# robingg1/PoseTraj

Measured on AMD Instinct MI355X. Metric: denoised frames/sec, higher is better.
Workload: dtype f16; 1 GPU; SVD-img2vid U-Net + controlnet_sdv, 14x576x1024, 25 Euler steps, CFG, 1 clip per GPU (BASELINE configs[2]); weights=random-init at full SVD dimensions (1524.6 M + 682.0 M params), output_finite=True, hipgraph=True, two_streams=True, rccl_world_size=1, weight_broadcast_collectives=0

## Files before the change

posetraj_amd/csrc/norm.hip:

```cpp
#include "pt_common.h"

namespace {

constexpr int GN_TX = 32, GN_TY = 8, GN_SLOTS = 36;

__global__ __launch_bounds__(256) void gn_partial_kernel(const f16* __restrict__ x0, const f16* __restrict__ x1,
                                                         int C0, int C1, int groups, int64_t rows_per_sample,
                                                         int rows_per_slab, float* __restrict__ part) {
    __shared__ float red[GN_TY][GN_TX * 8 * 2];
    __shared__ float chan[256 * 2];
    const int tx = threadIdx.x & 31, ty = threadIdx.x >> 5;
    const int slab = blockIdx.x, strip = blockIdx.y, sample = blockIdx.z;
    const int Ctot = C0 + C1, cg = Ctot / groups;
    const int c = strip * 256 + tx * 8;
    float s[8], q[8];
#pragma unroll
    for (int j = 0; j < 8; ++j) { s[j] = 0.f; q[j] = 0.f; }
    if (c < Ctot) {
        float pv[8];
#pragma unroll
        for (int j = 0; j < 8; ++j) pv[j] = pt_gn_pivot(x0, x1, C0, C1, rows_per_sample, sample, (c + j) / cg * cg);
        const f16* src; int ld, co;
        if (c < C0) { src = x0; ld = C0; co = c; } else { src = x1; ld = C1; co = c - C0; }
        const int64_t r0 = (int64_t)slab * rows_per_slab;
        int64_t r1 = r0 + rows_per_slab; if (r1 > rows_per_sample) r1 = rows_per_sample;
        const f16* base = src + ((int64_t)sample * rows_per_sample) * ld + co;
        int64_t r = r0 + ty;
        for (; r + 3 * GN_TY < r1; r += 4 * GN_TY) {
            f16x8 v[4];
#pragma unroll
            for (int u = 0; u < 4; ++u) v[u] = *(const f16x8*)(base + (r + u * GN_TY) * ld);
#pragma unroll
            for (int u = 0; u < 4; ++u)
#pragma unroll
                for (int j = 0; j < 8; ++j) { const float f = (float)v[u][j] - pv[j]; s[j] += f; q[j] += f * f; }
        }
        for (; r < r1; r += GN_TY) {
            const f16x8 v = *(const f16x8*)(base + r * ld);
#pragma unroll
            for (int j = 0; j < 8; ++j) { const float f = (float)v[j] - pv[j]; s[j] += f; q[j] += f * f; }
        }
    }
#pragma unroll
    for (int j = 0; j < 8; ++j) { red[ty][(tx * 8 + j) * 2] = s[j]; red[ty][(tx * 8 + j) * 2 + 1] = q[j]; }
    __syncthreads();
    for (int i = threadIdx.x; i < 256 * 2; i += 256) {
        float a = 0.f;
#pragma unroll
        for (int y = 0; y < GN_TY; ++y) a += red[y][i];
        chan[i] = a;
    }
    __syncthreads();
    const int c_lo = strip * 256, c_hi = (c_lo + 256 < Ctot) ? c_lo + 256 : Ctot;
    const int g_lo = c_lo / cg, g_hi = (c_hi - 1) / cg;
    const int ng = g_hi - g_lo + 1;
    if ((int)threadIdx.x < 2 * ng) {
        const int g = g_lo + (threadIdx.x >> 1), which = threadIdx.x & 1;
        int a0 = g * cg, a1 = a0 + cg;
        if (a0 < c_lo) a0 = c_lo;
        if (a1 > c_hi) a1 = c_hi;
        float acc = 0.f;
        for (int ch = a0; ch < a1; ++ch) acc += chan[(ch - c_lo) * 2 + which];
        part[((((int64_t)sample * gridDim.x + slab) * gridDim.y + strip) * GN_SLOTS + (g - g_lo)) * 2 + which] = acc;
    }
}

__device__ __forceinline__ void gn_fold_sample(const float* __restrict__ part, const f16* __restrict__ x0, const f16* __restrict__ x1,
                                               int C0, int C1, int sample, int nslabs, int nstrips, int groups,
                                               int64_t rows_per_sample, float eps, float* grp) {
    const int Ctot = C0 + C1, cg = Ctot / groups;
    const int sub = threadIdx.x & 7;
    for (int g = threadIdx.x >> 3; g < groups; g += blockDim.x >> 3) {
        float s = 0.f, q = 0.f;
        const int ch0 = g * cg, ch1 = ch0 + cg - 1;
        const float pg = pt_gn_pivot(x0, x1, C0, C1, rows_per_sample, sample, ch0);
        for (int strip = ch0 / 256; strip <= ch1 / 256; ++strip) {
            const int g_lo = (strip * 256) / cg;
            const float* base = part + ((int64_t)sample * nslabs * nstrips + strip) * GN_SLOTS * 2 + (g - g_lo) * 2;
            const int64_t step = (int64_t)nstrips * GN_SLOTS * 2;
            int sl = sub;
            for (; sl + 24 < nslabs; sl += 32) {
                const f32x2 e0 = *(const f32x2*)(base + sl * step), e1 = *(const f32x2*)(base + (sl + 8) * step);
                const f32x2 e2 = *(const f32x2*)(base + (sl + 16) * step), e3 = *(const f32x2*)(base + (sl + 24) * step);
                s += e0[0]; q += e0[1]; s += e1[0]; q += e1[1]; s += e2[0]; q += e2[1]; s += e3[0]; q += e3[1];
            }
            for (; sl < nslabs; sl += 8) {
                const float* e = base + sl * step;
                s += e[0]; q += e[1];
            }
        }
#pragma unroll
        for (int o = 1; o < 8; o <<= 1) { s += __shfl_xor(s, o); q += __shfl_xor(q, o); }
        if (sub == 0) {
            const double cnt = (double)rows_per_sample * cg;
            const double d = (double)s / cnt;
            double var = (double)q / cnt - d * d;
            if (var < 0.0) var = 0.0;
            grp[4 * g] = pg;
            grp[4 * g + 1] = (float)d;
            grp[4 * g + 2] = (float)(1.0 / sqrt(var + (double)eps));
        }
    }
}

__global__ __launch_bounds__(256) void gn_apply_kernel(const f16* __restrict__ x0, const f16* __restrict__ x1, int C0,
                                                       int C1, int rows_per_sample, int rows_per_block,
                                                       const float* __restrict__ part, int nslabs, int nstrips, int groups,
                                                       float eps, const f16* __restrict__ gamma, const f16* __restrict__ beta,
                                                       int silu, f16* __restrict__ y) {
    extern __shared__ __attribute__((aligned(16))) float s_ab[];
    __shared__ float grp[4 * 32];
    const int Ctot = C0 + C1, CH = Ctot >> 3;
    f16* const s_pv = (f16*)(s_ab + 2 * Ctot);
    const int sample = blockIdx.y;
    const int r0 = blockIdx.x * rows_per_block;
    const int r1 = min(r0 + rows_per_block, rows_per_sample);
    gn_fold_sample(part, x0, x1, C0, C1, sample, nslabs, nstrips, groups, rows_per_sample, eps, grp);
    __syncthreads();
    {
        const int cg = Ctot / groups;
        for (int c = threadIdx.x; c < Ctot; c += 256) {
            const int g = c / cg;
            const float a = grp[4 * g + 2] * (float)gamma[c];
            s_ab[2 * c] = a;
            s_ab[2 * c + 1] = (float)beta[c] - grp[4 * g + 1] * a;
            s_pv[c] = (f16)grp[4 * g];
        }
    }
    __syncthreads();
    const int64_t base_row = (int64_t)sample * rows_per_sample;
    const int dr = 256 / CH, dc = 256 - dr * CH;
    int row = r0 + (int)threadIdx.x / CH, c = (int)threadIdx.x % CH;
    auto advance = [&](int& rw, int& cc) {
        rw += dr; cc += dc;
        if (cc >= CH) { cc -= CH; ++rw; }
    };
    auto load = [&](int rw, int cc) -> f16x8 {
        const int ch = cc * 8;
        const int64_t grow = base_row + rw;
        return ch < C0 ? *(const f16x8*)(x0 + grow * C0 + ch) : *(const f16x8*)(x1 + grow * C1 + (ch - C0));
    };
    auto finish = [&](int rw, int cc, const f16x8& v) {
        const int ch = cc * 8;
        const f32x4* abp = (const f32x4*)(s_ab + ch * 2);
        const f16x8 pv = *(const f16x8*)(s_pv + ch);
        f16x8 o;
#pragma unroll
        for (int h = 0; h < 4; ++h) {
            const f32x4 k = abp[h];
            float u0 = ((float)v[2 * h] - (float)pv[2 * h]) * k[0] + k[1], u1 = ((float)v[2 * h + 1] - (float)pv[2 * h + 1]) * k[2] + k[3];
            if (silu) { u0 = pt_silu(u0); u1 = pt_silu(u1); }
            o[2 * h] = (f16)u0; o[2 * h + 1] = (f16)u1;
        }
        *(f16x8*)(y + (base_row + rw) * Ctot + ch) = o;
    };
    for (;;) {
        int rw[4], cc[4];
        rw[0] = row; cc[0] = c;
#pragma unroll
        for (int u = 1; u < 4; ++u) { rw[u] = rw[u - 1]; cc[u] = cc[u - 1]; advance(rw[u], cc[u]); }
        if (rw[3] >= r1) break;
        f16x8 v[4];
#pragma unroll
        for (int u = 0; u < 4; ++u) v[u] = load(rw[u], cc[u]);
#pragma unroll
        for (int u = 0; u < 4; ++u) finish(rw[u], cc[u], v[u]);
        row = rw[3]; c = cc[3];
        advance(row, c);
    }
    for (; row < r1; advance(row, c)) finish(row, c, load(row, c));
}

template <int NCH>
__global__ __launch_bounds__(256) void layernorm_kernel(const f16* __restrict__ x, int64_t M, int C,
                                                        const f16* __restrict__ vec, int ldv, int vec_mode, int vG,
                                                        const f16* __restrict__ gamma, const f16* __restrict__ beta,
                                                        float eps, f16* __restrict__ y) {
    const int lane = threadIdx.x & 63;
    const int64_t row = (int64_t)blockIdx.x * 4 + (threadIdx.x >> 6);
    if (row >= M) return;
    const int CH = C >> 3;
    float v[NCH][8];
    float sum = 0.f;
    const f16* vrow = vec_mode ? vec + (int64_t)(row / vG) * ldv : nullptr;
#pragma unroll
// ... 80 lines not shown
    if (!ok) return;
#pragma unroll
    for (int k = 0; k < CPL; ++k) {
        const int ch = l + LPR * k;
        const f16x8 g = *(const f16x8*)(gamma + ch * 8), b = *(const f16x8*)(beta + ch * 8);
        f16x8 o;
#pragma unroll
        for (int j = 0; j < 8; ++j) o[j] = (f16)((v[k][j] - mean) * rstd * (float)g[j] + (float)b[j]);
        *(f16x8*)(y + row * C + ch * 8) = o;
    }
}

int slab_rows(int64_t rows_per_sample, int nstrips, int n_samples) {
    int64_t target_slabs = 2048 / ((int64_t)nstrips * n_samples);
    if (target_slabs < 1) target_slabs = 1;
    if (target_slabs > 1024) target_slabs = 1024;
    int64_t rows = (rows_per_sample + target_slabs - 1) / target_slabs;
    if (rows < 64) rows = 64;
    rows = (rows + 7) / 8 * 8;
    return (int)rows;
}

}

extern "C" int64_t pt_groupnorm_scratch_floats(int64_t rows_total, int32_t C, int32_t n_samples) {
    const int64_t rps = rows_total / (n_samples > 0 ? n_samples : 1);
    const int nstrips = (C + 255) / 256;
    const int rows = slab_rows(rps, nstrips, n_samples);
    const int64_t nslabs = (rps + rows - 1) / rows;
    return (int64_t)n_samples * nslabs * nstrips * GN_SLOTS * 2;
}

extern "C" int pt_groupnorm_stats(const void* x0, const void* x1, int32_t C0, int32_t C1, int32_t groups,
                                  int64_t rows_per_sample, int32_t n_samples, float* partials, void* stream) {
    const int Ctot = C0 + C1;
    PT_CHECK(x0 && partials, "pt_groupnorm_stats: null pointer");
    PT_CHECK(C0 % 8 == 0 && C1 % 8 == 0 && groups > 0 && groups <= 32 && Ctot % groups == 0 && Ctot / groups >= 2,
             "pt_groupnorm_stats: C0=%d C1=%d groups=%d", C0, C1, groups);
    PT_CHECK((C1 == 0) == (x1 == nullptr), "pt_groupnorm_stats: x1/C1 mismatch");
    PT_CHECK(rows_per_sample > 0 && n_samples > 0, "pt_groupnorm_stats: empty input");
    const int nstrips = (Ctot + 255) / 256;
    const int rows = slab_rows(rows_per_sample, nstrips, n_samples);
    const int nslabs = (int)((rows_per_sample + rows - 1) / rows);
    PT_CHECK(n_samples <= 65535 && nstrips <= 65535, "pt_groupnorm_stats: grid too large");
    hipLaunchKernelGGL(gn_partial_kernel, dim3(nslabs, nstrips, n_samples), dim3(256), 0, (hipStream_t)stream, (const f16*)x0,
                       (const f16*)x1, C0, C1, groups, rows_per_sample, rows, partials);
    PT_LAUNCH_CHECK("pt_groupnorm_stats");
    return 0;
}

extern "C" int pt_groupnorm_apply(const void* x0, const void* x1, int32_t C0, int32_t C1, int32_t groups,
                                  int64_t rows_per_sample, int32_t n_samples, float eps, const void* gamma,
                                  const void* beta, const float* partials, int32_t silu, void* y, void* stream) {
    PT_CHECK(x0 && gamma && beta && partials && y, "pt_groupnorm_apply: null pointer");
    PT_CHECK(C0 % 8 == 0 && C1 % 8 == 0, "pt_groupnorm_apply: channels must be multiples of 8");
    const int Ctot = C0 + C1;
    PT_CHECK(Ctot >= 8 && Ctot <= 4096, "pt_groupnorm_apply: %d channels unsupported (8 .. 4096)", Ctot);
    PT_CHECK(groups > 0 && groups <= 32 && Ctot % groups == 0 && Ctot / groups >= 2, "pt_groupnorm_apply: C=%d groups=%d", Ctot, groups);
    PT_CHECK(rows_per_sample > 0 && rows_per_sample < (1ll << 31) && n_samples > 0 && n_samples <= 65535, "pt_groupnorm_apply: bad sizes");
    const int nstrips = (Ctot + 255) / 256;
    const int srows = slab_rows(rows_per_sample, nstrips, n_samples);
    const int nslabs = (int)((rows_per_sample + srows - 1) / srows);
    int64_t per_sample = 4096 / n_samples;
    if (per_sample < 1) per_sample = 1;
    int64_t rows_per_block = (rows_per_sample + per_sample - 1) / per_sample;
    const int64_t total_chunks = rows_per_sample * n_samples * (Ctot >> 3);
    const int min_chunks = total_chunks < (int64_t)256 * 32 * 1024 ? 8 : 32;
    const int64_t min_rows = (256 * min_chunks + (Ctot >> 3) - 1) / (Ctot >> 3);
    if (rows_per_block < min_rows) rows_per_block = min_rows;
    const unsigned bx = (unsigned)((rows_per_sample + rows_per_block - 1) / rows_per_block);
    hipLaunchKernelGGL(gn_apply_kernel, dim3(bx, (unsigned)n_samples), dim3(256), (size_t)Ctot * 10, (hipStream_t)stream,
                       (const f16*)x0, (const f16*)x1, C0, C1, (int)rows_per_sample, (int)rows_per_block, partials, nslabs,
                       nstrips, groups, eps, (const f16*)gamma, (const f16*)beta, silu, (f16*)y);
    PT_LAUNCH_CHECK("pt_groupnorm_apply");
    return 0;
}

extern "C" int pt_layernorm_f16(const void* x, int64_t M, int32_t C, const void* vec, int32_t ldv, int32_t vec_mode,
                                int32_t vG, const void* gamma, const void* beta, float eps, void* y, void* stream) {
    PT_CHECK(x && gamma && beta && y, "pt_layernorm_f16: null pointer");
    PT_CHECK(C % 8 == 0 && C <= 2048, "pt_layernorm_f16: C=%d must be a multiple of 8 and <= 2048", C);
    PT_CHECK(vec_mode == 0 || (vec_mode == 1 && vec && vG > 0 && ldv % 8 == 0), "pt_layernorm_f16: bad vec arguments");
    hipStream_t s = (hipStream_t)stream;
#define LN_NARROW(LPR, CPL)                                                                                            \
    do {                                                                                                               \
        const int64_t rpb = 4 * (64 / LPR);                                                                            \
        hipLaunchKernelGGL((layernorm_narrow_kernel<LPR, CPL>), dim3((unsigned)((M + rpb - 1) / rpb)), dim3(256), 0, s, \
                           (const f16*)x, M, C, (const f16*)vec, ldv, vec_mode, vG, (const f16*)gamma, (const f16*)beta, \
// ... 3 lines not shown
    } while (0)
    if (C == 320) LN_NARROW(8, 5);
    if (C == 640) LN_NARROW(16, 5);
    if (C == 1280) LN_NARROW(32, 5);
#undef LN_NARROW
    const unsigned blocks = (unsigned)((M + 3) / 4);
    const int nch = ((C >> 3) + 63) / 64;
#define LN_LAUNCH(NCH)                                                                                              \
    hipLaunchKernelGGL(layernorm_kernel<NCH>, dim3(blocks), dim3(256), 0, s, (const f16*)x, M, C, (const f16*)vec, \
                       ldv, vec_mode, vG, (const f16*)gamma, (const f16*)beta, eps, (f16*)y)
    if (nch == 1) LN_LAUNCH(1); else if (nch == 2) LN_LAUNCH(2); else if (nch == 3) LN_LAUNCH(3); else LN_LAUNCH(4);
#undef LN_LAUNCH
    PT_LAUNCH_CHECK("pt_layernorm_f16");
    return 0;
}
```

posetraj_amd/hip.py:

```python
from __future__ import annotations

import ctypes as C
import os
import re
import subprocess

HERE = os.path.dirname(os.path.abspath(__file__))
CSRC = os.path.join(HERE, "csrc")
LIB_PATH = os.path.abspath(os.environ["PT_LIB"]) if os.environ.get("PT_LIB") else os.path.join(HERE, "libposetraj_hip.so")
SOURCES = ["api.hip", "igemm.hip", "ffn.hip", "lnlin.hip", "norm.hip", "attn.hip", "attn_general.hip", "elementwise.hip", "vae.hip", "vae_f32.hip", "clip.hip", "raster.hip", "train.hip", "gemm.hip", "backward.hip", "attn_bwd.hip", "batch.hip", "control.hip", "sampler.hip"]
HEADERS = ["pt_common.h", "igemm_tail.h", "pt_fold.h"]
HEADER = os.path.join(HERE, "..", "include", "posetraj_hip.h")
STRUCT_CLASSES = {"pt_igemm_params": "IgemmParams", "pt_ffn_params": "FfnParams", "pt_lnlin_params": "LnLinParams",
                  "pt_conv_f32_params": "ConvF32Params", "pt_gemm_params": "GemmParams"}
OPTIM_HEADER = os.path.join(HERE, "..", "include", "posetraj_optim.h")
OPTIM_STRUCT_CLASSES = {"pt_adam8_segment": "Adam8Segment"}
DET_HEADER = os.path.join(HERE, "..", "include", "posetraj_det.h")
TEMPORAL_HEADER = os.path.join(HERE, "..", "include", "posetraj_temporal.h")
BATCH_HEADER = os.path.join(HERE, "..", "include", "posetraj_batch.h")
CONTROL_HEADER = os.path.join(HERE, "..", "include", "posetraj_control.h")
SAMPLER_HEADER = os.path.join(HERE, "..", "include", "posetraj_sampler.h")

_lib = _checked = None

_SCALARS = {"int": C.c_int, "int32_t": C.c_int32, "int64_t": C.c_int64, "float": C.c_float, "double": C.c_double}
_TYPE = r"(?:const\s+)?\w+\s*\*?"
_DECL = re.compile(r"""\s*(?: typedef\s+struct\s+(?P<tag>\w+)\s*\{(?P<body>[^{}]*)\}\s*(?P=tag)\s*;
                            | (?P<ret>%s)\s*\b(?P<fn>pt[odtbcs]?_[a-z0-9_]+)\s*\((?P<params>[^()]*)\)\s*;
                            | extern\s+"C"\s*\{ | \} )""" % _TYPE, re.X)
_FIELD = re.compile(r"(%s)\s*\b(\w+(?:\s*,\s*\w+)*)" % _TYPE)


def _ctype(spelling: str, structs: dict, returned: bool = False):
    m = re.fullmatch(r"(const\s+)?(\w+)\s*(\*)?", spelling)
    const, base, ptr = m.groups() if m else (None, None, None)
    if not ptr and not const and base in _SCALARS:
        return _SCALARS[base]
    if ptr and const and base in structs:
        return C.POINTER(structs[base])
    if ptr and const and base == "char" and returned:
        return C.c_char_p
    if ptr and (base == "void" or base in _SCALARS):
        return C.c_void_p
# ... 19 lines not shown
    structs, protos, pos = dict(known_structs or {}), {}, 0
    while text[pos:].strip():
        m = _DECL.match(text, pos)
        if not m:
            raise ValueError(f"posetraj_hip.h: cannot read the declaration {text[pos:].strip().split(';')[0][:200]!r}")
        if m.group("tag"):
            tag = m.group("tag")
            if tag not in struct_classes:
                raise ValueError(f"posetraj_hip.h: struct {tag!r} has no class name in posetraj_amd.hip.STRUCT_CLASSES")
            fields = [(n, _ctype(t, structs)) for t, n in _declarators(m.group("body"), ";")]
            structs[tag] = type(struct_classes[tag], (C.Structure,), {"_fields_": fields, "__doc__": f"``{tag}`` of include/posetraj_hip.h."})
        elif m.group("fn"):
            params = m.group("params").strip()
            protos[m.group("fn")] = (" ".join(m.group("ret").split()), [] if params == "void" else [t for t, _ in _declarators(params, ",")])
        pos = m.end()
    named = re.findall(r"pt[odtbcs]?_[a-z0-9_]+\s*\(", text)
    if len(named) != len(protos):
        raise ValueError(f"posetraj_hip.h: {len(named)} names are followed by '(' but {len(protos)} prototypes were read")
    return int(version.group(1)), {k: v for k, v in structs.items() if k not in (known_structs or {})}, protos


with open(HEADER) as _f:
    ABI_VERSION, _STRUCTS, PROTOTYPES = _parse_header(_f.read())
IgemmParams, FfnParams, LnLinParams, ConvF32Params, GemmParams = (_STRUCTS[tag] for tag in STRUCT_CLASSES)
SIGNATURES = {name: (_ctype(ret, _STRUCTS, returned=True), [_ctype(t, _STRUCTS) for t in params]) for name, (ret, params) in PROTOTYPES.items()}
with open(OPTIM_HEADER) as _f:
    OPTIM_ABI_VERSION, _OPTIM_STRUCTS, OPTIM_PROTOTYPES = _parse_header(_f.read(), OPTIM_STRUCT_CLASSES, "PT_OPTIM_ABI_VERSION")
Adam8Segment = _OPTIM_STRUCTS["pt_adam8_segment"]
OPTIM_SIGNATURES = {name: (_ctype(ret, _OPTIM_STRUCTS, returned=True), [_ctype(t, _OPTIM_STRUCTS) for t in params])
                    for name, (ret, params) in OPTIM_PROTOTYPES.items()}
with open(DET_HEADER) as _f:
    DET_ABI_VERSION, _, DET_PROTOTYPES = _parse_header(_f.read(), {}, "PT_DET_ABI_VERSION", _STRUCTS)
DET_SIGNATURES = {name: (_ctype(ret, _STRUCTS, returned=True), [_ctype(t, _STRUCTS) for t in params]) for name, (ret, params) in DET_PROTOTYPES.items()}
with open(TEMPORAL_HEADER) as _f:
    TEMPORAL_ABI_VERSION, _, TEMPORAL_PROTOTYPES = _parse_header(_f.read(), {}, "PT_TEMPORAL_ABI_VERSION", _STRUCTS)
TEMPORAL_SIGNATURES = {name: (_ctype(ret, _STRUCTS, returned=True), [_ctype(t, _STRUCTS) for t in params]) for name, (ret, params) in TEMPORAL_PROTOTYPES.items()}
with open(BATCH_HEADER) as _f:
    BATCH_ABI_VERSION, _, BATCH_PROTOTYPES = _parse_header(_f.read(), {}, "PT_BATCH_ABI_VERSION", _STRUCTS)
BATCH_SIGNATURES = {name: (_ctype(ret, _STRUCTS, returned=True), [_ctype(t, _STRUCTS) for t in params]) for name, (ret, params) in BATCH_PROTOTYPES.items()}
with open(CONTROL_HEADER) as _f:
    CONTROL_ABI_VERSION, _, CONTROL_PROTOTYPES = _parse_header(_f.read(), {}, "PT_CONTROL_ABI_VERSION", _STRUCTS)
CONTROL_SIGNATURES = {name: (_ctype(ret, _STRUCTS, returned=True), [_ctype(t, _STRUCTS) for t in params]) for name, (ret, params) in CONTROL_PROTOTYPES.items()}
with open(SAMPLER_HEADER) as _f:
    SAMPLER_ABI_VERSION, _, SAMPLER_PROTOTYPES = _parse_header(_f.read(), {}, "PT_SAMPLER_ABI_VERSION", _STRUCTS)
SAMPLER_SIGNATURES = {name: (_ctype(ret, _STRUCTS, returned=True), [_ctype(t, _STRUCTS) for t in params]) for name, (ret, params) in SAMPLER_PROTOTYPES.items()}


def build(force: bool = False, verbose: bool = False) -> str:
    if os.environ.get("PT_LIB"):
        raise RuntimeError("posetraj_amd.hip.build: PT_LIB is set (A/B against another library); unset it to build the tree's own")
    from concurrent.futures import ThreadPoolExecutor
    headers = [os.path.join(CSRC, h) for h in HEADERS] + [HEADER, OPTIM_HEADER, DET_HEADER, TEMPORAL_HEADER, BATCH_HEADER, CONTROL_HEADER, SAMPLER_HEADER]
    hdr_time = max(os.path.getmtime(h) for h in headers)
    objdir = os.path.join(CSRC, "_obj")
    os.makedirs(objdir, exist_ok=True)
    hipcc = os.environ.get("HIPCC", "/opt/rocm/bin/hipcc")
    jobs = []
    for name in SOURCES:
        src, obj = os.path.join(CSRC, name), os.path.join(objdir, name + ".o")
        rem = obj + ".remarks"
        if force or not (os.path.exists(obj) and os.path.exists(rem)) or os.path.getmtime(obj) < max(os.path.getmtime(src), hdr_time):
            jobs.append((src, obj, rem))

    def compile_one(job):
        src, obj, rem = job
        cmd = [hipcc, "--offload-arch=gfx950", "-O3", "-std=c++17", "-fPIC", "-Rpass-analysis=kernel-resource-usage", "-c", src, "-o", obj]
        if verbose:
# ... 40 lines not shown
        m = re.search(r"Function Name: (\S+)", line)
        if m:
            cur = out.setdefault(m.group(1), {})
            continue
        m = re.search(r"remark:\s+([A-Za-z][A-Za-z ]*?)(?: \[[^\]]*\])?:\s+(\d+)", line)
        if m and cur is not None:
            cur[m.group(1).strip()] = int(m.group(2))
    if out:
        with open(RESOURCES_PATH, "w") as f:
            json.dump(out, f, indent=0, sort_keys=True)


def source_digest() -> str:
    import hashlib
    h = hashlib.sha256()
    for path in sorted([os.path.join(CSRC, s) for s in SOURCES + HEADERS] + [HEADER, OPTIM_HEADER, DET_HEADER, TEMPORAL_HEADER, BATCH_HEADER, CONTROL_HEADER, SAMPLER_HEADER]):
        with open(path, "rb") as f:
            h.update(os.path.basename(path).encode() + b"\0" + f.read())
    return h.hexdigest()


def _load(errcheck=None):
    if not os.path.exists(LIB_PATH):
        raise RuntimeError(f"{LIB_PATH} not found: run `python -c 'import __graft_entry__ as g; g.build()'` "
                           "(posetraj_amd has no CPU or PyTorch fallback path)")
    L = C.CDLL(LIB_PATH)
    for sigs, protos in ((SIGNATURES, PROTOTYPES), (OPTIM_SIGNATURES, OPTIM_PROTOTYPES), (DET_SIGNATURES, DET_PROTOTYPES),
                         (TEMPORAL_SIGNATURES, TEMPORAL_PROTOTYPES), (BATCH_SIGNATURES, BATCH_PROTOTYPES), (CONTROL_SIGNATURES, CONTROL_PROTOTYPES),
                         (SAMPLER_SIGNATURES, SAMPLER_PROTOTYPES)):
        for name, (res, args) in sigs.items():
            fn = getattr(L, name)
            fn.restype, fn.argtypes = res, args
            if errcheck is not None and protos[name][0] == "int" and name not in ("pt_abi_version", "pto_abi_version", "ptd_abi_version", "ptt_abi_version", "ptb_abi_version", "ptc_abi_version", "pts_abi_version"):
                fn.errcheck = errcheck
    if (L.pt_abi_version() != ABI_VERSION or L.pto_abi_version() != OPTIM_ABI_VERSION or L.ptd_abi_version() != DET_ABI_VERSION
            or L.ptt_abi_version() != TEMPORAL_ABI_VERSION or L.ptb_abi_version() != BATCH_ABI_VERSION or L.ptc_abi_version() != CONTROL_ABI_VERSION
            or L.pts_abi_version() != SAMPLER_ABI_VERSION):
        raise RuntimeError(f"libposetraj_hip.so ABI {L.pt_abi_version()} / optimizer extension {L.pto_abi_version()} / deterministic extension "
                           f"{L.ptd_abi_version()} / long-clip extension {L.ptt_abi_version()} / clip-batch extension {L.ptb_abi_version()} / control-weight extension "
                           f"{L.ptc_abi_version()} / sampler extension {L.pts_abi_version()} != expected {ABI_VERSION} / {OPTIM_ABI_VERSION} / {DET_ABI_VERSION} / "
                           f"{TEMPORAL_ABI_VERSION} / {BATCH_ABI_VERSION} / {CONTROL_ABI_VERSION} / {SAMPLER_ABI_VERSION}; rebuild")
    return L


def lib():
    global _lib
    if _lib is None:
        _lib = _load()
    return _lib


def checked():
    global _checked
    if _checked is None:
        _checked = _load(_raise_on_status)
    return _checked
# ... 12 lines not shown
```

posetraj_amd/ops.py:

```python
from __future__ import annotations

import ctypes as C
from dataclasses import dataclass
from typing import Optional

import torch

from . import hip

WIDE_KINDS = frozenset(("sc", "xs", "rb"))
WIDE_STREAM = True


_inplace_writes = {}


def _attach_lo(hi: torch.Tensor, lo: torch.Tensor) -> None:
    hi.lo = lo
    hi.lo_gen = _inplace_writes.get(hi.data_ptr(), 0)


def wview(t: torch.Tensor, *shape) -> torch.Tensor:
    v = t.view(*shape)
    lo = getattr(t, "lo", None)
# ... 261 lines not shown
    return out


def groupnorm(x0: torch.Tensor, gamma: torch.Tensor, beta: torch.Tensor, *, rows_per_sample: int, n_samples: int,
              eps: float, silu: bool, x1: Optional[torch.Tensor] = None, groups: int = 32) -> torch.Tensor:
    ensure_ready(x0.device)
    _need(x0, "x0")
    C0 = x0.shape[-1]
    C1 = x1.shape[-1] if x1 is not None else 0
    Ct = C0 + C1
    rows = rows_per_sample * n_samples
    L = hip.checked()
    nfl = L.pt_groupnorm_scratch_floats(rows, Ct, n_samples)
    partials = torch.empty(nfl, dtype=torch.float32, device=x0.device)
    st = _stream()
    L.pt_groupnorm_stats(x0.data_ptr(), _ptr(x1), C0, C1, groups, rows_per_sample, n_samples, partials.data_ptr(), st)
    y = torch.empty((rows, Ct), dtype=torch.float16, device=x0.device)
    L.pt_groupnorm_apply(x0.data_ptr(), _ptr(x1), C0, C1, groups, rows_per_sample, n_samples, float(eps),
                         gamma.data_ptr(), beta.data_ptr(), partials.data_ptr(), 1 if silu else 0, y.data_ptr(), st)
    return y


def layernorm(x: torch.Tensor, gamma: torch.Tensor, beta: torch.Tensor, eps: float = 1e-5, *,
              vec: Optional[torch.Tensor] = None, vG: int = 0) -> torch.Tensor:
    _need(x, "x")
    M, Cc = x.shape
    y = torch.empty_like(x)
    hip.checked().pt_layernorm_f16(x.data_ptr(), M, Cc, _ptr(vec), (vec.stride(0) if vec is not None else 0),
                                   1 if vec is not None else 0, vG, gamma.data_ptr(), beta.data_ptr(), float(eps),
                                   y.data_ptr(), _stream())
    return y

# ... 316 lines not shown
```

Baseline: 4.247 frames/s.

## Add planned GroupNorm entry with single-launch register-resident form

Adds a new GroupNorm entry point that picks a form per shape. For small per-sample channel strips it uses a resident kernel: one block of 1024 threads loads its strip into registers, computes mean and variance in two passes, and writes normalized output, so input is read once in a single launch. Otherwise it keeps the two-launch stats/apply path, now with a deeper unrolled stats loop, a fixed-width fold, and gamma/beta plus the first input tile prefetched before the stats fold. Large register tiles and few blocks may hurt occupancy on some shapes.

```diff
diff --git a/include/posetraj_norm.h b/include/posetraj_norm.h
--- /dev/null
+++ b/include/posetraj_norm.h
@@ -0,0 +1,30 @@
+#ifndef POSETRAJ_NORM_H
+#define POSETRAJ_NORM_H
+
+#include <stdint.h>
+
+#include "posetraj_hip.h"
+
+#ifdef __cplusplus
+extern "C" {
+#endif
+
+#define PT_NORM_ABI_VERSION 1
+
+int ptn_abi_version(void);
+
+int ptn_groupnorm_f16(const void* x0, const void* x1, int32_t C0, int32_t C1, int32_t groups, int64_t rows_per_sample,
+                      int32_t n_samples, float eps, const void* gamma, const void* beta, float* scratch, int32_t silu, void* y,
+                      void* stream);
+
+int ptn_groupnorm_plan(int32_t C0, int32_t C1, int32_t groups, int64_t rows_per_sample, int32_t n_samples, int32_t* plan);
+
+int ptn_groupnorm_force_form(int32_t form);
+
+int ptn_groupnorm_force_limits(int64_t unit_bytes, int32_t min_units);
+
+#ifdef __cplusplus
+}
+#endif
+
+#endif
diff --git a/posetraj_amd/csrc/norm.hip b/posetraj_amd/csrc/norm.hip
--- a/posetraj_amd/csrc/norm.hip
+++ b/posetraj_amd/csrc/norm.hip
@@ -1,9 +1,24 @@
 #include "pt_common.h"
+#include "../../include/posetraj_norm.h"
 
 namespace {
 
 constexpr int GN_TX = 32, GN_TY = 8, GN_SLOTS = 36;
-
+constexpr int GN_FOLD_T = 8, GN_FOLD_L = 8, GN_MAX_SLABS = GN_FOLD_T * GN_FOLD_L;
+constexpr int GN_DEEP_ROWS = 512;
+
+template <int U>
+__device__ __forceinline__ void gn_accumulate(const f16* base, int ld, int64_t r, const float (&pv)[8], float (&s)[8], float (&q)[8]) {
+    f16x8 v[U];
+#pragma unroll
+    for (int u = 0; u < U; ++u) v[u] = *(const f16x8*)(base + (r + u * GN_TY) * ld);
+#pragma unroll
+    for (int u = 0; u < U; ++u)
+#pragma unroll
+        for (int j = 0; j < 8; ++j) { const float f = (float)v[u][j] - pv[j]; s[j] += f; q[j] += f * f; }
+}
+
+template <bool DEEP>
 __global__ __launch_bounds__(256) void gn_partial_kernel(const f16* __restrict__ x0, const f16* __restrict__ x1,
                                                          int C0, int C1, int groups, int64_t rows_per_sample,
                                                          int rows_per_slab, float* __restrict__ part) {
@@ -26,20 +41,10 @@
         int64_t r1 = r0 + rows_per_slab; if (r1 > rows_per_sample) r1 = rows_per_sample;
         const f16* base = src + ((int64_t)sample * rows_per_sample) * ld + co;
         int64_t r = r0 + ty;
-        for (; r + 3 * GN_TY < r1; r += 4 * GN_TY) {
-            f16x8 v[4];
-#pragma unroll
-            for (int u = 0; u < 4; ++u) v[u] = *(const f16x8*)(base + (r + u * GN_TY) * ld);
-#pragma unroll
-            for (int u = 0; u < 4; ++u)
-#pragma unroll
-                for (int j = 0; j < 8; ++j) { const float f = (float)v[u][j] - pv[j]; s[j] += f; q[j] += f * f; }
-        }
-        for (; r < r1; r += GN_TY) {
-            const f16x8 v = *(const f16x8*)(base + r * ld);
-#pragma unroll
-            for (int j = 0; j < 8; ++j) { const float f = (float)v[j] - pv[j]; s[j] += f; q[j] += f * f; }
-        }
+        if (DEEP)
+            for (; r + 7 * GN_TY < r1; r += 8 * GN_TY) gn_accumulate<8>(base, ld, r, pv, s, q);
+        for (; r + 3 * GN_TY < r1; r += 4 * GN_TY) gn_accumulate<4>(base, ld, r, pv, s, q);
+        for (; r < r1; r += GN_TY) gn_accumulate<1>(base, ld, r, pv, s, q);
     }
 #pragma unroll
     for (int j = 0; j < 8; ++j) { red[ty][(tx * 8 + j) * 2] = s[j]; red[ty][(tx * 8 + j) * 2 + 1] = q[j]; }
@@ -65,6 +70,7 @@
     }
 }
 
+template <int FOLD_L>
 __device__ __forceinline__ void gn_fold_sample(const float* __restrict__ part, const f16* __restrict__ x0, const f16* __restrict__ x1,
                                                int C0, int C1, int sample, int nslabs, int nstrips, int groups,
                                                int64_t rows_per_sample, float eps, float* grp) {
@@ -77,17 +83,16 @@
         for (int strip = ch0 / 256; strip <= ch1 / 256; ++strip) {
             const int g_lo = (strip * 256) / cg;
             const float* base = part + ((int64_t)sample * nslabs * nstrips + strip) * GN_SLOTS * 2 + (g - g_lo) * 2;
-            const int64_t step = (int64_t)nstrips * GN_SLOTS * 2;
-            int sl = sub;
-            for (; sl + 24 < nslabs; sl += 32) {
-                const f32x2 e0 = *(const f32x2*)(base + sl * step), e1 = *(const f32x2*)(base + (sl + 8) * step);
-                const f32x2 e2 = *(const f32x2*)(base + (sl + 16) * step), e3 = *(const f32x2*)(base + (sl + 24) * step);
-                s += e0[0]; q += e0[1]; s += e1[0]; q += e1[1]; s += e2[0]; q += e2[1]; s += e3[0]; q += e3[1];
+            const int step = nstrips * GN_SLOTS * 2;
+            f32x2 e[FOLD_L];
+#pragma unroll
+            for (int k = 0; k < FOLD_L; ++k) {
+                const int sl = sub + GN_FOLD_T * k;
+                e[k] = *(const f32x2*)(base + (sl < nslabs ? sl : nslabs - 1) * step);
             }
-            for (; sl < nslabs; sl += 8) {
-                const float* e = base + sl * step;
-                s += e[0]; q += e[1];
-            }
+#pragma unroll
+            for (int k = 0; k < FOLD_L; ++k)
+                if (sub + GN_FOLD_T * k < nslabs) { s += e[k][0]; q += e[k][1]; }
         }
 #pragma unroll
         for (int o = 1; o < 8; o <<= 1) { s += __shfl_xor(s, o); q += __shfl_xor(q, o); }
@@ -103,6 +108,7 @@
     }
 }
 
+template <bool PRE_X, int FOLD_L>
 __global__ __launch_bounds__(256) void gn_apply_kernel(const f16* __restrict__ x0, const f16* __restrict__ x1, int C0,
                                                        int C1, int rows_per_sample, int rows_per_block,
                                                        const float* __restrict__ part, int nslabs, int nstrips, int groups,
@@ -115,19 +121,6 @@
     const int sample = blockIdx.y;
     const int r0 = blockIdx.x * rows_per_block;
     const int r1 = min(r0 + rows_per_block, rows_per_sample);
-    gn_fold_sample(part, x0, x1, C0, C1, sample, nslabs, nstrips, groups, rows_per_sample, eps, grp);
-    __syncthreads();
-    {
-        const int cg = Ctot / groups;
-        for (int c = threadIdx.x; c < Ctot; c += 256) {
-            const int g = c / cg;
-            const float a = grp[4 * g + 2] * (float)gamma[c];
-            s_ab[2 * c] = a;
-            s_ab[2 * c + 1] = (float)beta[c] - grp[4 * g + 1] * a;
-            s_pv[c] = (f16)grp[4 * g];
-        }
-    }
-    __syncthreads();
     const int64_t base_row = (int64_t)sample * rows_per_sample;
     const int dr = 256 / CH, dc = 256 - dr * CH;
     int row = r0 + (int)threadIdx.x / CH, c = (int)threadIdx.x % CH;
@@ -154,21 +147,185 @@
         }
         *(f16x8*)(y + (base_row + rw) * Ctot + ch) = o;
     };
-    for (;;) {
-        int rw[4], cc[4];
+    int rw[4], cc[4];
+    f16x8 v[4];
+    auto first_trip = [&]() {
         rw[0] = row; cc[0] = c;
 #pragma unroll
         for (int u = 1; u < 4; ++u) { rw[u] = rw[u - 1]; cc[u] = cc[u - 1]; advance(rw[u], cc[u]); }
-        if (rw[3] >= r1) break;
-        f16x8 v[4];
-#pragma unroll
-        for (int u = 0; u < 4; ++u) v[u] = load(rw[u], cc[u]);
-#pragma unroll
-        for (int u = 0; u < 4; ++u) finish(rw[u], cc[u], v[u]);
-        row = rw[3]; c = cc[3];
-        advance(row, c);
-    }
-    for (; row < r1; advance(row, c)) finish(row, c, load(row, c));
+#pragma unroll
+        for (int u = 0; u < 4; ++u)
+            if (rw[u] < r1) v[u] = load(rw[u], cc[u]);
+    };
+    if (PRE_X) first_trip();
+    constexpr int GN_AB_PRE = 5;
+    f16x2 gm[GN_AB_PRE], bt[GN_AB_PRE];
+#pragma unroll
+    for (int k = 0; k < GN_AB_PRE; ++k) {
+        const int ch = 2 * (int)threadIdx.x + 512 * k;
+        if (ch < Ctot) { gm[k] = *(const f16x2*)(gamma + ch); bt[k] = *(const f16x2*)(beta + ch); }
+    }
+    gn_fold_sample<FOLD_L>(part, x0, x1, C0, C1, sample, nslabs, nstrips, groups, rows_per_sample, eps, grp);
+    __syncthreads();
+    {
+        const int cg = Ctot / groups;
+        auto fill = [&](int ch, f16 gv, f16 bv) {
+            const int g = ch / cg;
+            const float a = grp[4 * g + 2] * (float)gv;
+            s_ab[2 * ch] = a;
+            s_ab[2 * ch + 1] = (float)bv - grp[4 * g + 1] * a;
+            s_pv[ch] = (f16)grp[4 * g];
+        };
+#pragma unroll
+        for (int k = 0; k < GN_AB_PRE; ++k) {
+            const int ch = 2 * (int)threadIdx.x + 512 * k;
+            if (ch < Ctot) { fill(ch, gm[k][0], bt[k][0]); fill(ch + 1, gm[k][1], bt[k][1]); }
+        }
+        for (int ch = (int)threadIdx.x + 512 * GN_AB_PRE; ch < Ctot; ch += 256) fill(ch, gamma[ch], beta[ch]);
+    }
+    __syncthreads();
+    if (!PRE_X) first_trip();
+    if (rw[3] < r1) {
+        for (;;) {
+#pragma unroll
+            for (int u = 0; u < 4; ++u) finish(rw[u], cc[u], v[u]);
+            rw[0] = rw[3]; cc[0] = cc[3];
+            advance(rw[0], cc[0]);
+#pragma unroll
+            for (int u = 1; u < 4; ++u) { rw[u] = rw[u - 1]; cc[u] = cc[u - 1]; advance(rw[u], cc[u]); }
+            if (rw[3] >= r1) break;
+#pragma unroll
+            for (int u = 0; u < 4; ++u) v[u] = load(rw[u], cc[u]);
+        }
+        for (row = rw[0], c = cc[0]; row < r1; advance(row, c)) finish(row, c, load(row, c));
+    } else {
+#pragma unroll
+        for (int u = 0; u < 4; ++u)
+            if (rw[u] < r1) finish(rw[u], cc[u], v[u]);
+    }
+}
+
+constexpr int GN_RES_T = 1024, GN_RES_MAXCH = 12, GN_RES_MAXW = 1024;
+
+template <int NCH>
+__global__ __launch_bounds__(GN_RES_T) void gn_resident_kernel(const f16* __restrict__ x0, const f16* __restrict__ x1, int C0, int C1,
+                                                               int groups, int rows, int W, float eps, const f16* __restrict__ gamma,
+                                                               const f16* __restrict__ beta, int silu, f16* __restrict__ y) {
+    __shared__ __attribute__((aligned(16))) float red[GN_RES_T * 8];
+    __shared__ float red2[GN_RES_T];
+    __shared__ float chan[GN_RES_MAXW];
+    __shared__ __attribute__((aligned(16))) float chd[GN_RES_MAXW], cha[GN_RES_MAXW], chb[GN_RES_MAXW];
+    const int Ctot = C0 + C1, cg = Ctot / groups;
+    const int sample = blockIdx.y;
+    const int c_lo = blockIdx.x * W, Ws = min(W, Ctot - c_lo), CHs = Ws >> 3;
+    const int RL = GN_RES_T / CHs, RLu = min(RL, rows);
+    const int t = threadIdx.x, rl = t / CHs, col = t - rl * CHs;
+    const bool live = rl < RLu;
+    const int ch = c_lo + col * 8;
+    float gv = 0.f, bv = 0.f;
+    if (t < Ws) { gv = (float)gamma[c_lo + t]; bv = (float)beta[c_lo + t]; }
+    const f16* base = x0;
+    int ld = 0;
+    float pv[8];
+#pragma unroll
+    for (int j = 0; j < 8; ++j) pv[j] = 0.f;
+    if (live) {
+        if (ch < C0) { ld = C0; base = x0 + (int64_t)sample * rows * C0 + ch; } else { ld = C1; base = x1 + (int64_t)sample * rows * C1 + (ch - C0); }
+#pragma unroll
+        for (int j = 0; j < 8; ++j) pv[j] = pt_gn_pivot(x0, x1, C0, C1, rows, sample, (ch + j) / cg * cg);
+    }
+    f16x8 v[NCH];
+#pragma unroll
+    for (int k = 0; k < NCH; ++k) {
+        const int r = rl + k * RL;
+        if (live && r < rows) v[k] = *(const f16x8*)(base + (int64_t)r * ld);
+        else {
+#pragma unroll
+            for (int j = 0; j < 8; ++j) v[k][j] = (f16)0.f;
+        }
+    }
+    const int P = min(RLu, GN_RES_T / Ws);
+    const float cnt = (float)rows * (float)cg;
+    auto channel_sums = [&](const float (&acc)[8]) {
+        if (live) {
+            *(f32x4*)(red + rl * Ws + col * 8) = f32x4{acc[0], acc[1], acc[2], acc[3]};
+            *(f32x4*)(red + rl * Ws + col * 8 + 4) = f32x4{acc[4], acc[5], acc[6], acc[7]};
+        }
+        __syncthreads();
+        if (t < P * Ws) {
+            const int p = t / Ws, c = t - p * Ws;
+            float a = 0.f;
+            for (int r = p; r < RLu; r += P) a += red[r * Ws + c];
+            red2[t] = a;
+        }
+        __syncthreads();
+        if (t < Ws) {
+            float a = 0.f;
+            for (int p = 0; p < P; ++p) a += red2[p * Ws + t];
+            chan[t] = a;
+        }
+        __syncthreads();
+    };
+    auto group_sum = [&]() -> float {
+        const int g0 = t / cg * cg;
+        float a = 0.f;
+        for (int i = 0; i < cg; ++i) a += chan[g0 + i];
+        return a;
+    };
+    float acc[8];
+#pragma unroll
+    for (int j = 0; j < 8; ++j) acc[j] = 0.f;
+#pragma unroll
+    for (int k = 0; k < NCH; ++k)
+        if (rl + k * RL < rows)
+#pragma unroll
+            for (int j = 0; j < 8; ++j) acc[j] += (float)v[k][j] - pv[j];
+    channel_sums(acc);
+    if (t < Ws) chd[t] = group_sum() / cnt;
+    __syncthreads();
+    float d[8];
+    {
+        const f32x4 d0 = *(const f32x4*)(chd + col * 8), d1 = *(const f32x4*)(chd + col * 8 + 4);
+#pragma unroll
+        for (int j = 0; j < 4; ++j) { d[j] = d0[j]; d[4 + j] = d1[j]; }
+    }
+#pragma unroll
+    for (int j = 0; j < 8; ++j) acc[j] = 0.f;
+#pragma unroll
+    for (int k = 0; k < NCH; ++k)
+        if (rl + k * RL < rows)
+#pragma unroll
+            for (int j = 0; j < 8; ++j) { const float f = ((float)v[k][j] - pv[j]) - d[j]; acc[j] += f * f; }
+    channel_sums(acc);
+    if (t < Ws) {
+        const double var = (double)group_sum() / (double)cnt;
+        cha[t] = (float)(1.0 / sqrt(var + (double)eps)) * gv;
+        chb[t] = bv;
+    }
+    __syncthreads();
+    if (!live) return;
+    float a[8], b[8];
+    {
+        const f32x4 a0 = *(const f32x4*)(cha + col * 8), a1 = *(const f32x4*)(cha + col * 8 + 4);
+        const f32x4 b0 = *(const f32x4*)(chb + col * 8), b1 = *(const f32x4*)(chb + col * 8 + 4);
+#pragma unroll
+        for (int j = 0; j < 4; ++j) { a[j] = a0[j]; a[4 + j] = a1[j]; b[j] = b0[j]; b[4 + j] = b1[j]; }
+    }
+    f16* out = y + (int64_t)sample * rows * Ctot + ch;
+#pragma unroll
+    for (int k = 0; k < NCH; ++k) {
+        const int r = rl + k * RL;
+        if (r < rows) {
+            f16x8 o;
+#pragma unroll
+            for (int j = 0; j < 8; ++j) {
+                float u = (((float)v[k][j] - pv[j]) - d[j]) * a[j] + b[j];
+                if (silu) u = pt_silu(u);
+                o[j] = (f16)u;
+            }
+            *(f16x8*)(out + (int64_t)r * Ctot) = o;
+        }
+    }
 }
 
 template <int NCH>
@@ -279,11 +436,81 @@
 int slab_rows(int64_t rows_per_sample, int nstrips, int n_samples) {
     int64_t target_slabs = 2048 / ((int64_t)nstrips * n_samples);
     if (target_slabs < 1) target_slabs = 1;
-    if (target_slabs > 1024) target_slabs = 1024;
+    if (target_slabs > GN_MAX_SLABS) target_slabs = GN_MAX_SLABS;
     int64_t rows = (rows_per_sample + target_slabs - 1) / target_slabs;
     if (rows < 64) rows = 64;
     rows = (rows + 7) / 8 * 8;
     return (int)rows;
+}
+
+constexpr int64_t GN_RES_UNIT_BYTES = 192 * 1024;
+constexpr int GN_RES_MIN_UNITS = 112;
+constexpr int GN_RES_PLAN_MINW = 160, GN_RES_PLAN_MAXW = 320;
+enum { GN_FORM_AUTO = 0, GN_FORM_TWO_LAUNCH = 1, GN_FORM_RESIDENT = 2 };
+int g_gn_force_form = GN_FORM_AUTO;
+int64_t g_gn_unit_bytes = GN_RES_UNIT_BYTES;
+int g_gn_min_units = GN_RES_MIN_UNITS;
+int g_gn_minw = GN_RES_PLAN_MINW, g_gn_maxw = GN_RES_PLAN_MAXW;
+
+struct GnPlan {
+    int form, strip, nstrips, units, chunks, slabs, slab_rows, last_strip;
+};
+
+int gn_gcd(int a, int b) { return b ? gn_gcd(b, a % b) : a; }
+
+int gn_resident_chunks(int64_t rows, int W) {
+    if (W > GN_RES_MAXW) return 0;
+    const int64_t rl = GN_RES_T / (W >> 3);
+    const int64_t need = (rows + rl - 1) / rl;
+    return need <= GN_RES_MAXCH ? (int)need : 0;
+}
+
+bool gn_resident_geometry(int64_t rows, int Ctot, int groups, int* strip) {
+    const int cg = Ctot / groups;
+    const int unit = cg / gn_gcd(cg, 8) * 8;
+    int m = (Ctot < g_gn_maxw ? Ctot : g_gn_maxw) / unit;
+    while (m >= 1 && !(rows * m * unit * 2 <= g_gn_unit_bytes && gn_resident_chunks(rows, m * unit))) --m;
+    if (m < 1 || m * unit < g_gn_minw) return false;
+    const int widest = m * unit;
+    const int line = unit / gn_gcd(unit, 64) * 64;
+    if (line <= widest) { *strip = widest / line * line; return true; }
+    const int n = (Ctot + widest - 1) / widest;
+    *strip = ((Ctot + n - 1) / n + unit - 1) / unit * unit;
+    return true;
+}
+
+bool gn_args_ok(const char* who, int C0, int C1, int groups, int64_t rows_per_sample, int n_samples) {
+    const int Ctot = C0 + C1;
+    if (C0 <= 0 || C1 < 0 || C0 % 8 != 0 || C1 % 8 != 0 || Ctot > 4096) { pt_set_error("%s: C0=%d C1=%d must be multiples of 8, at most 4096 together", who, C0, C1); return false; }
+    if (groups <= 0 || groups > 32 || Ctot % groups != 0 || Ctot / groups < 2) { pt_set_error("%s: C=%d groups=%d", who, Ctot, groups); return false; }
+    if (rows_per_sample <= 0 || rows_per_sample >= (1ll << 31) || n_samples <= 0 || n_samples > 65535) { pt_set_error("%s: bad sizes", who); return false; }
+    return true;
+}
+
+int gn_plan(const char* who, int C0, int C1, int groups, int64_t rows_per_sample, int n_samples, GnPlan* p) {
+    const int Ctot = C0 + C1;
+    const int stat_strips = (Ctot + 255) / 256;
+    p->slab_rows = slab_rows(rows_per_sample, stat_strips, n_samples);
+    p->slabs = (int)((rows_per_sample + p->slab_rows - 1) / p->slab_rows);
+    p->form = GN_FORM_TWO_LAUNCH;
+    p->strip = 256; p->nstrips = stat_strips; p->last_strip = Ctot - (stat_strips - 1) * 256;
+    p->units = p->slabs * stat_strips * n_samples;
+    p->chunks = 0;
+    int W = 0;
+    const bool legal = g_gn_force_form != GN_FORM_TWO_LAUNCH && gn_resident_geometry(rows_per_sample, Ctot, groups, &W);
+    if (g_gn_force_form == GN_FORM_RESIDENT && !legal) {
+        pt_set_error("%s: no resident form for %lld rows x %d channels in %d groups (unit limit %lld bytes)", who, (long long)rows_per_sample,
+                     Ctot, groups, (long long)g_gn_unit_bytes);
+        return 1;
+    }
+    if (!legal) return 0;
+    const int n = (Ctot + W - 1) / W;
+    if (g_gn_force_form == GN_FORM_AUTO && (int64_t)n * n_samples < g_gn_min_units) return 0;
+    p->form = GN_FORM_RESIDENT;
+    p->strip = W; p->nstrips = n; p->last_strip = Ctot - (n - 1) * W;
+    p->units = n * n_samples;
+    p->chunks = gn_resident_chunks(rows_per_sample, W);
+    return 0;
 }
 
 }
@@ -308,8 +535,12 @@
     const int rows = slab_rows(rows_per_sample, nstrips, n_samples);
     const int nslabs = (int)((rows_per_sample + rows - 1) / rows);
     PT_CHECK(n_samples <= 65535 && nstrips <= 65535, "pt_groupnorm_stats: grid too large");
-    hipLaunchKernelGGL(gn_partial_kernel, dim3(nslabs, nstrips, n_samples), dim3(256), 0, (hipStream_t)stream, (const f16*)x0,
-                       (const f16*)x1, C0, C1, groups, rows_per_sample, rows, partials);
+    if (rows >= GN_DEEP_ROWS)
+        hipLaunchKernelGGL(gn_partial_kernel<true>, dim3(nslabs, nstrips, n_samples), dim3(256), 0, (hipStream_t)stream, (const f16*)x0,
+                           (const f16*)x1, C0, C1, groups, rows_per_sample, rows, partials);
+    else
+        hipLaunchKernelGGL(gn_partial_kernel<false>, dim3(nslabs, nstrips, n_samples), dim3(256), 0, (hipStream_t)stream, (const f16*)x0,
+                           (const f16*)x1, C0, C1, groups, rows_per_sample, rows, partials);
     PT_LAUNCH_CHECK("pt_groupnorm_stats");
     return 0;
 }
@@ -334,9 +565,17 @@
     const int64_t min_rows = (256 * min_chunks + (Ctot >> 3) - 1) / (Ctot >> 3);
     if (rows_per_block < min_rows) rows_per_block = min_rows;
     const unsigned bx = (unsigned)((rows_per_sample + rows_per_block - 1) / rows_per_block);
-    hipLaunchKernelGGL(gn_apply_kernel, dim3(bx, (unsigned)n_samples), dim3(256), (size_t)Ctot * 10, (hipStream_t)stream,
-                       (const f16*)x0, (const f16*)x1, C0, C1, (int)rows_per_sample, (int)rows_per_block, partials, nslabs,
-                       nstrips, groups, eps, (const f16*)gamma, (const f16*)beta, silu, (f16*)y);
+#define GN_APPLY_LAUNCH(PRE_X, FOLD_L)                                                                                              \
+    hipLaunchKernelGGL((gn_apply_kernel<PRE_X, FOLD_L>), dim3(bx, (unsigned)n_samples), dim3(256), (size_t)Ctot * 10, (hipStream_t)stream, \
+                       (const f16*)x0, (const f16*)x1, C0, C1, (int)rows_per_sample, (int)rows_per_block, partials, nslabs, nstrips,   \
+                       groups, eps, (const f16*)gamma, (const f16*)beta, silu, (f16*)y)
+    static_assert(GN_MAX_SLABS == 64, "the fold depths below cover 8, 32 and 64 slabs");
+    if (min_chunks == 32) {
+        if (nslabs <= GN_FOLD_T) GN_APPLY_LAUNCH(true, 1); else if (nslabs <= 4 * GN_FOLD_T) GN_APPLY_LAUNCH(true, 4); else GN_APPLY_LAUNCH(true, 8);
+    } else {
+        if (nslabs <= GN_FOLD_T) GN_APPLY_LAUNCH(false, 1); else if (nslabs <= 4 * GN_FOLD_T) GN_APPLY_LAUNCH(false, 4); else GN_APPLY_LAUNCH(false, 8);
+    }
+#undef GN_APPLY_LAUNCH
     PT_LAUNCH_CHECK("pt_groupnorm_apply");
     return 0;
 }
@@ -370,3 +609,54 @@
     PT_LAUNCH_CHECK("pt_layernorm_f16");
     return 0;
 }
+
+extern "C" int ptn_abi_version(void) { return PT_NORM_ABI_VERSION; }
+
+extern "C" int ptn_groupnorm_force_form(int32_t form) {
+    PT_CHECK(form == GN_FORM_AUTO || form == GN_FORM_TWO_LAUNCH || form == GN_FORM_RESIDENT, "ptn_groupnorm_force_form: form %d (0 automatic, 1 two launches, 2 resident)", form);
+    g_gn_force_form = form;
+    return 0;
+}
+
+extern "C" int ptn_groupnorm_force_limits(int64_t unit_bytes, int32_t min_units) {
+    PT_CHECK(unit_bytes >= 0 && min_units >= 0, "ptn_groupnorm_force_limits: negative limit");
+    g_gn_unit_bytes = unit_bytes ? unit_bytes : GN_RES_UNIT_BYTES;
+    g_gn_min_units = unit_bytes ? min_units : GN_RES_MIN_UNITS;
+    g_gn_minw = unit_bytes ? 8 : GN_RES_PLAN_MINW;
+    g_gn_maxw = unit_bytes ? GN_RES_MAXW : GN_RES_PLAN_MAXW;
+    return 0;
+}
+
+extern "C" int ptn_groupnorm_plan(int32_t C0, int32_t C1, int32_t groups, int64_t rows_per_sample, int32_t n_samples, int32_t* plan) {
+    PT_CHECK(plan, "ptn_groupnorm_plan: null pointer");
+    if (!gn_args_ok("ptn_groupnorm_plan", C0, C1, groups, rows_per_sample, n_samples)) return 1;
+    GnPlan p;
+    if (gn_plan("ptn_groupnorm_plan", C0, C1, groups, rows_per_sample, n_samples, &p)) return 1;
+    plan[0] = p.form; plan[1] = p.strip; plan[2] = p.nstrips; plan[3] = p.units;
+    plan[4] = p.chunks; plan[5] = p.slabs; plan[6] = p.slab_rows; plan[7] = p.last_strip;
+    return 0;
+}
+
+extern "C" int ptn_groupnorm_f16(const void* x0, const void* x1, int32_t C0, int32_t C1, int32_t groups, int64_t rows_per_sample,
+                                 int32_t n_samples, float eps, const void* gamma, const void* beta, float* scratch, int32_t silu, void* y,
+                                 void* stream) {
+    PT_CHECK(x0 && gamma && beta && y, "ptn_groupnorm_f16: null pointer");
+    PT_CHECK((C1 == 0) == (x1 == nullptr), "ptn_groupnorm_f16: x1/C1 mismatch");
+    if (!gn_args_ok("ptn_groupnorm_f16", C0, C1, groups, rows_per_sample, n_samples)) return 1;
+    GnPlan p;
+    if (gn_plan("ptn_groupnorm_f16", C0, C1, groups, rows_per_sample, n_samples, &p)) return 1;
+    if (p.form == GN_FORM_TWO_LAUNCH) {
+        PT_CHECK(scratch, "ptn_groupnorm_f16: the two-launch form needs the scratch of pt_groupnorm_scratch_floats");
+        if (pt_groupnorm_stats(x0, x1, C0, C1, groups, rows_per_sample, n_samples, scratch, stream)) return 1;
+        return pt_groupnorm_apply(x0, x1, C0, C1, groups, rows_per_sample, n_samples, eps, gamma, beta, scratch, silu, y, stream);
+    }
+    const dim3 grid((unsigned)p.nstrips, (unsigned)n_samples);
+#define GN_RES_LAUNCH(NCH)                                                                                                          \
+    hipLaunchKernelGGL(gn_resident_kernel<NCH>, grid, dim3(GN_RES_T), 0, (hipStream_t)stream, (const f16*)x0, (const f16*)x1, C0, C1, \
+                       groups, (int)rows_per_sample, p.strip, eps, (const f16*)gamma, (const f16*)beta, silu, (f16*)y)
+    if (p.chunks <= 1) GN_RES_LAUNCH(1); else if (p.chunks <= 2) GN_RES_LAUNCH(2); else if (p.chunks <= 4) GN_RES_LAUNCH(4);
+    else if (p.chunks <= 8) GN_RES_LAUNCH(8); else GN_RES_LAUNCH(12);
+#undef GN_RES_LAUNCH
+    PT_LAUNCH_CHECK("ptn_groupnorm_f16");
+    return 0;
+}
diff --git a/posetraj_amd/hip.py b/posetraj_amd/hip.py
--- a/posetraj_amd/hip.py
+++ b/posetraj_amd/hip.py
@@ -20,13 +20,14 @@
 BATCH_HEADER = os.path.join(HERE, "..", "include", "posetraj_batch.h")
 CONTROL_HEADER = os.path.join(HERE, "..", "include", "posetraj_control.h")
 SAMPLER_HEADER = os.path.join(HERE, "..", "include", "posetraj_sampler.h")
+NORM_HEADER = os.path.join(HERE, "..", "include", "posetraj_norm.h")
 
 _lib = _checked = None
 
 _SCALARS = {"int": C.c_int, "int32_t": C.c_int32, "int64_t": C.c_int64, "float": C.c_float, "double": C.c_double}
 _TYPE = r"(?:const\s+)?\w+\s*\*?"
 _DECL = re.compile(r"""\s*(?: typedef\s+struct\s+(?P<tag>\w+)\s*\{(?P<body>[^{}]*)\}\s*(?P=tag)\s*;
-                            | (?P<ret>%s)\s*\b(?P<fn>pt[odtbcs]?_[a-z0-9_]+)\s*\((?P<params>[^()]*)\)\s*;
+                            | (?P<ret>%s)\s*\b(?P<fn>pt[odtbcsn]?_[a-z0-9_]+)\s*\((?P<params>[^()]*)\)\s*;
                             | extern\s+"C"\s*\{ | \} )""" % _TYPE, re.X)
 _FIELD = re.compile(r"(%s)\s*\b(\w+(?:\s*,\s*\w+)*)" % _TYPE)
 
@@ -76,7 +77,7 @@
             params = m.group("params").strip()
             protos[m.group("fn")] = (" ".join(m.group("ret").split()), [] if params == "void" else [t for t, _ in _declarators(params, ",")])
         pos = m.end()
-    named = re.findall(r"pt[odtbcs]?_[a-z0-9_]+\s*\(", text)
+    named = re.findall(r"pt[odtbcsn]?_[a-z0-9_]+\s*\(", text)
     if len(named) != len(protos):
         raise ValueError(f"posetraj_hip.h: {len(named)} names are followed by '(' but {len(protos)} prototypes were read")
     return int(version.group(1)), {k: v for k, v in structs.items() if k not in (known_structs or {})}, protos
@@ -106,13 +107,16 @@
 with open(SAMPLER_HEADER) as _f:
     SAMPLER_ABI_VERSION, _, SAMPLER_PROTOTYPES = _parse_header(_f.read(), {}, "PT_SAMPLER_ABI_VERSION", _STRUCTS)
 SAMPLER_SIGNATURES = {name: (_ctype(ret, _STRUCTS, returned=True), [_ctype(t, _STRUCTS) for t in params]) for name, (ret, params) in SAMPLER_PROTOTYPES.items()}
+with open(NORM_HEADER) as _f:
+    NORM_ABI_VERSION, _, NORM_PROTOTYPES = _parse_header(_f.read(), {}, "PT_NORM_ABI_VERSION", _STRUCTS)
+NORM_SIGNATURES = {name: (_ctype(ret, _STRUCTS, returned=True), [_ctype(t, _STRUCTS) for t in params]) for name, (ret, params) in NORM_PROTOTYPES.items()}
 
 
 def build(force: bool = False, verbose: bool = False) -> str:
     if os.environ.get("PT_LIB"):
         raise RuntimeError("posetraj_amd.hip.build: PT_LIB is set (A/B against another library); unset it to build the tree's own")
     from concurrent.futures import ThreadPoolExecutor
-    headers = [os.path.join(CSRC, h) for h in HEADERS] + [HEADER, OPTIM_HEADER, DET_HEADER, TEMPORAL_HEADER, BATCH_HEADER, CONTROL_HEADER, SAMPLER_HEADER]
+    headers = [os.path.join(CSRC, h) for h in HEADERS] + [HEADER, OPTIM_HEADER, DET_HEADER, TEMPORAL_HEADER, BATCH_HEADER, CONTROL_HEADER, SAMPLER_HEADER, NORM_HEADER]
     hdr_time = max(os.path.getmtime(h) for h in headers)
     objdir = os.path.join(CSRC, "_obj")
     os.makedirs(objdir, exist_ok=True)
@@ -183,7 +187,7 @@
 def source_digest() -> str:
     import hashlib
     h = hashlib.sha256()
-    for path in sorted([os.path.join(CSRC, s) for s in SOURCES + HEADERS] + [HEADER, OPTIM_HEADER, DET_HEADER, TEMPORAL_HEADER, BATCH_HEADER, CONTROL_HEADER, SAMPLER_HEADER]):
+    for path in sorted([os.path.join(CSRC, s) for s in SOURCES + HEADERS] + [HEADER, OPTIM_HEADER, DET_HEADER, TEMPORAL_HEADER, BATCH_HEADER, CONTROL_HEADER, SAMPLER_HEADER, NORM_HEADER]):
         with open(path, "rb") as f:
             h.update(os.path.basename(path).encode() + b"\0" + f.read())
     return h.hexdigest()
@@ -196,19 +200,19 @@
     L = C.CDLL(LIB_PATH)
     for sigs, protos in ((SIGNATURES, PROTOTYPES), (OPTIM_SIGNATURES, OPTIM_PROTOTYPES), (DET_SIGNATURES, DET_PROTOTYPES),
                          (TEMPORAL_SIGNATURES, TEMPORAL_PROTOTYPES), (BATCH_SIGNATURES, BATCH_PROTOTYPES), (CONTROL_SIGNATURES, CONTROL_PROTOTYPES),
-                         (SAMPLER_SIGNATURES, SAMPLER_PROTOTYPES)):
+                         (SAMPLER_SIGNATURES, SAMPLER_PROTOTYPES), (NORM_SIGNATURES, NORM_PROTOTYPES)):
         for name, (res, args) in sigs.items():
             fn = getattr(L, name)
             fn.restype, fn.argtypes = res, args
-            if errcheck is not None and protos[name][0] == "int" and name not in ("pt_abi_version", "pto_abi_version", "ptd_abi_version", "ptt_abi_version", "ptb_abi_version", "ptc_abi_version", "pts_abi_version"):
+            if errcheck is not None and protos[name][0] == "int" and name not in ("pt_abi_version", "pto_abi_version", "ptd_abi_version", "ptt_abi_version", "ptb_abi_version", "ptc_abi_version", "pts_abi_version", "ptn_abi_version"):
                 fn.errcheck = errcheck
     if (L.pt_abi_version() != ABI_VERSION or L.pto_abi_version() != OPTIM_ABI_VERSION or L.ptd_abi_version() != DET_ABI_VERSION
             or L.ptt_abi_version() != TEMPORAL_ABI_VERSION or L.ptb_abi_version() != BATCH_ABI_VERSION or L.ptc_abi_version() != CONTROL_ABI_VERSION
-            or L.pts_abi_version() != SAMPLER_ABI_VERSION):
+            or L.pts_abi_version() != SAMPLER_ABI_VERSION or L.ptn_abi_version() != NORM_ABI_VERSION):
         raise RuntimeError(f"libposetraj_hip.so ABI {L.pt_abi_version()} / optimizer extension {L.pto_abi_version()} / deterministic extension "
                            f"{L.ptd_abi_version()} / long-clip extension {L.ptt_abi_version()} / clip-batch extension {L.ptb_abi_version()} / control-weight extension "
-                           f"{L.ptc_abi_version()} / sampler extension {L.pts_abi_version()} != expected {ABI_VERSION} / {OPTIM_ABI_VERSION} / {DET_ABI_VERSION} / "
-                           f"{TEMPORAL_ABI_VERSION} / {BATCH_ABI_VERSION} / {CONTROL_ABI_VERSION} / {SAMPLER_ABI_VERSION}; rebuild")
+                           f"{L.ptc_abi_version()} / sampler extension {L.pts_abi_version()} / GroupNorm extension {L.ptn_abi_version()} != expected {ABI_VERSION} / {OPTIM_ABI_VERSION} / {DET_ABI_VERSION} / "
+                           f"{TEMPORAL_ABI_VERSION} / {BATCH_ABI_VERSION} / {CONTROL_ABI_VERSION} / {SAMPLER_ABI_VERSION} / {NORM_ABI_VERSION}; rebuild")
     return L
 
 
diff --git a/posetraj_amd/ops.py b/posetraj_amd/ops.py
--- a/posetraj_amd/ops.py
+++ b/posetraj_amd/ops.py
@@ -299,8 +299,24 @@
     nfl = L.pt_groupnorm_scratch_floats(rows, Ct, n_samples)
     partials = torch.empty(nfl, dtype=torch.float32, device=x0.device)
     st = _stream()
+    y = torch.empty((rows, Ct), dtype=torch.float16, device=x0.device)
+    L.ptn_groupnorm_f16(x0.data_ptr(), _ptr(x1), C0, C1, groups, rows_per_sample, n_samples, float(eps),
+                        gamma.data_ptr(), beta.data_ptr(), partials.data_ptr(), 1 if silu else 0, y.data_ptr(), st)
+    return y
+
+
+def groupnorm_two_launch(x0: torch.Tensor, gamma: torch.Tensor, beta: torch.Tensor, *, rows_per_sample: int, n_samples: int,
+                         eps: float, silu: bool, x1: Optional[torch.Tensor] = None, groups: int = 32) -> torch.Tensor:
+    ensure_ready(x0.device)
+    _need(x0, "x0")
+    C0 = x0.shape[-1]
+    C1 = x1.shape[-1] if x1 is not None else 0
+    rows = rows_per_sample * n_samples
+    L = hip.checked()
+    partials = torch.empty(L.pt_groupnorm_scratch_floats(rows, C0 + C1, n_samples), dtype=torch.float32, device=x0.device)
+    st = _stream()
     L.pt_groupnorm_stats(x0.data_ptr(), _ptr(x1), C0, C1, groups, rows_per_sample, n_samples, partials.data_ptr(), st)
-    y = torch.empty((rows, Ct), dtype=torch.float16, device=x0.device)
+    y = torch.empty((rows, C0 + C1), dtype=torch.float16, device=x0.device)
     L.pt_groupnorm_apply(x0.data_ptr(), _ptr(x1), C0, C1, groups, rows_per_sample, n_samples, float(eps),
                          gamma.data_ptr(), beta.data_ptr(), partials.data_ptr(), 1 if silu else 0, y.data_ptr(), st)
     return y
```

Result: no change. 4.267 frames/s, median of 6 (+0.5%).
